# kscalelabs/kbot-joystick

Hardware: AMD Instinct MI355X
Metric: env-steps/sec (whole node), K-Bot joystick 8192 envs @1/2/4/8 MI355X (higher is better)
Workload: dtype f32; 1 GPU; kbot-headless, 8192 envs/GPU, flat ground, fixed joystick command (0.5,0,0), full iteration: 100-step rollout + PPO update (batch 512/GPU, 3 passes, LSTM hidden 256, depth 2); envs_per_gpu=8192, rollout_steps=100, batch_size_per_gpu=512, num_passes=3, hidden_size=256, deterministic_update=True, parallelism=env-sharded dp1, grad all-reduce per optimizer step

## Files before the change

### kbot-joystick_amd/csrc/kbj_gemm.h

```cpp
#pragma once
#include <hip/hip_runtime.h>
#include <algorithm>
#include <type_traits>
#include "kbj_ctx.h"

namespace kbj {

typedef float f32x16 __attribute__((ext_vector_type(16)));
typedef float f32x4 __attribute__((ext_vector_type(4)));

struct GemmArgs {
  const float* A; const float* B; float* C; const float* bias;
  int M, N, K;
  int lda, ldb, ldc;
  int beta;
  int splitk;
  const int* a_rows;
  const float* A2 = nullptr; const float* B2 = nullptr; int k1 = 0;
  float* C2 = nullptr; int n1 = 0, ldb2 = 0, ldc2 = 0;
  const int* a_idx = nullptr; int a_B = 0, a_N = 0;
  float* skws = nullptr;
  int x3 = 0;
};

constexpr int GEMM_BK = 32;
constexpr int GEMM_LDK = 36;

template <int ROWS, bool KC, int NTH>
struct GemmStage {
  static constexpr int NV = ROWS * 8 / NTH;
  static constexpr int RPP = NTH / 8;
  f32x4 v[NV];
  __device__ __forceinline__ void load_fast(const float* __restrict__ P, int ld, int r0, int k0) {
    const int tid = threadIdx.x;
    if (KC) {
      const int kq = tid & 7, rr = tid >> 3;
      const float* p = P + (size_t)(r0 + rr) * ld + k0 + 4 * kq;
#pragma unroll
      for (int i = 0; i < NV; ++i) v[i] = *reinterpret_cast<const f32x4*>(p + (size_t)(RPP * i) * ld);
    } else {
      constexpr int QPR = ROWS / 4, KROWS = NTH / QPR;
      const int rq = tid % QPR, kr0 = tid / QPR;
      const float* p = P + (size_t)(k0 + kr0) * ld + r0 + 4 * rq;
#pragma unroll
      for (int i = 0; i < NV; ++i) v[i] = *reinterpret_cast<const f32x4*>(p + (size_t)(KROWS * i) * ld);
    }
  }
  __device__ __forceinline__ void load(const float* __restrict__ P, int ld, int R, int r0, int k0, int kend, bool vec, const int* idx = nullptr, int iB = 0,
                                       int iN = 0) {
    const int tid = threadIdx.x;
    if (KC) {
      const int kq = tid & 7, rr = tid >> 3;
#pragma unroll
      for (int i = 0; i < NV; ++i) {
        int r = r0 + rr + RPP * i, k = k0 + 4 * kq;
        f32x4 x = {0, 0, 0, 0};
        if (r < R) {
          size_t base = (size_t)r * ld;
          if (idx) { const int t = r / iB; base = ((size_t)t * iN + idx[r - t * iB]) * ld; }
          if (vec && k + 3 < kend) x = *reinterpret_cast<const f32x4*>(P + base + k);
          else { for (int e = 0; e < 4; ++e) if (k + e < kend) x[e] = P[base + k + e]; }
        }
        v[i] = x;
      }
    } else {
      constexpr int QPR = ROWS / 4, KROWS = NTH / QPR;
      const int rq = tid % QPR, kr0 = tid / QPR;
#pragma unroll
      for (int i = 0; i < NV; ++i) {
        int k = k0 + kr0 + KROWS * i, r = r0 + 4 * rq;
        f32x4 x = {0, 0, 0, 0};
        if (k < kend) {
          size_t base = (size_t)k * ld;
          if (vec && r + 3 < R) x = *reinterpret_cast<const f32x4*>(P + base + r);
          else { for (int e = 0; e < 4; ++e) if (r + e < R) x[e] = P[base + r + e]; }
        }
        v[i] = x;
      }
    }
  }
  __device__ __forceinline__ void store(float* lds) const {
    const int tid = threadIdx.x;
    if (KC) {
      const int kq = tid & 7, rr = tid >> 3;
#pragma unroll
      for (int i = 0; i < NV; ++i) *reinterpret_cast<f32x4*>(lds + (rr + RPP * i) * GEMM_LDK + 4 * kq) = v[i];
    } else {
      constexpr int QPR = ROWS / 4, KROWS = NTH / QPR;
      const int rq = tid % QPR, kr0 = tid / QPR;
#pragma unroll
      for (int i = 0; i < NV; ++i) *reinterpret_cast<f32x4*>(lds + (kr0 + KROWS * i) * (ROWS + 4) + 4 * rq) = v[i];
    }
  }
};

struct GemmItem { int m0, n0, kbeg, kend, ks; const float* B; float* C; int ncols, ldb, ldc, ncol0; };
template <int BM, int BN>
__device__ __forceinline__ GemmItem gemm_item(const GemmArgs& g, int item, int tiles_n, int tiles_m, int per) {
  GemmItem it;
  int tn = item % tiles_n, r = item / tiles_n;
  int tm = r % tiles_m;
  it.ks = r / tiles_m;
  it.m0 = tm * BM; it.n0 = tn * BN;
  it.B = g.B; it.C = g.C; it.ncols = g.N; it.ldb = g.ldb; it.ldc = g.ldc; it.ncol0 = 0;
  if (g.n1 > 0) {
    if (it.n0 >= g.n1) {
      it.B = g.B2; it.C = g.C2; it.n0 -= g.n1; it.ncols = g.N - g.n1; it.ncol0 = g.n1;
      if (g.ldb2 > 0) it.ldb = g.ldb2;
      if (g.ldc2 > 0) it.ldc = g.ldc2;
    }
    else it.ncols = g.n1;
  }
  it.kbeg = it.ks * per;
  it.kend = min(g.K, it.kbeg + per);
  return it;
}

template <int MT, int NT, bool A_KC, bool B_KC, int WM = 2, int WN = 2>
__global__ __launch_bounds__(64 * WM * WN) void gemm_f32_kernel(GemmArgs g) {
  constexpr int BM = 32 * MT * WM, BN = 32 * NT * WN, NTH = 64 * WM * WN;
  constexpr int A_ELEMS = A_KC ? BM * GEMM_LDK : GEMM_BK * (BM + 4);
  constexpr int B_ELEMS = B_KC ? BN * GEMM_LDK : GEMM_BK * (BN + 4);
  constexpr int STAGE = A_ELEMS + B_ELEMS;
  extern __shared__ __attribute__((aligned(16))) float lds[];
  const int tid = threadIdx.x, lane = tid & 63, wave = tid >> 6;
  const int wr = wave / WN, wc = wave % WN;
  const int lr = lane & 31, lh = lane >> 5;
  const int tiles_n = (g.N + BN - 1) / BN, tiles_m = (g.M + BM - 1) / BM;
  const int sk = g.splitk > 1 ? g.splitk : 1;
  const int per = sk > 1 ? ((g.K + sk - 1) / sk + GEMM_BK - 1) / GEMM_BK * GEMM_BK : g.K;
  const int items = tiles_n * tiles_m * sk;
  const int item = (blockIdx.x & 7) * (gridDim.x >> 3) + (blockIdx.x >> 3);
  if (item >= items) return;
  const GemmItem cur = gemm_item<BM, BN>(g, item, tiles_n, tiles_m, per);
  if (cur.kbeg >= cur.kend) return;

  const bool a_vec = (g.lda & 3) == 0 && (((size_t)g.A & 15) == 0) && (((size_t)g.A2 & 15) == 0);
  const bool b_vec = (g.ldb & 3) == 0 && (g.ldb2 & 3) == 0 && (((size_t)g.B & 15) == 0) && (((size_t)g.B2 & 15) == 0);
  const bool rows_a = a_vec && cur.m0 + BM <= g.M, rows_b = b_vec && cur.n0 + BN <= cur.ncols;
  GemmStage<BM, A_KC, NTH> sa;
  GemmStage<BN, B_KC, NTH> sb;
  unsigned voa[GemmStage<BM, A_KC, NTH>::NV], vob[GemmStage<BN, B_KC, NTH>::NV];
  {
    if (A_KC) { const int kq = tid & 7, rr = tid >> 3;
#pragma unroll
      for (int i = 0; i < sa.NV; ++i) {
        size_t row = (size_t)(cur.m0 + rr + sa.RPP * i);
        if (g.a_idx && rows_a) {
          const int m = (int)row, t = m / g.a_B;
          row = (size_t)(t - cur.m0 / g.a_B) * g.a_N + g.a_idx[m - t * g.a_B];
        }
        voa[i] = (unsigned)((row * g.lda + 4 * kq) * 4);
      } }
    else { constexpr int QPR = BM / 4, KROWS = NTH / QPR; const int rq = tid % QPR, kr0 = tid / QPR;
#pragma unroll
      for (int i = 0; i < sa.NV; ++i) voa[i] = (unsigned)(((size_t)(kr0 + KROWS * i) * g.lda + cur.m0 + 4 * rq) * 4); }
    if (B_KC) { const int kq = tid & 7, rr = tid >> 3;
#pragma unroll
      for (int i = 0; i < sb.NV; ++i) vob[i] = (unsigned)(((size_t)(cur.n0 + rr + sb.RPP * i) * cur.ldb + 4 * kq) * 4); }
    else { constexpr int QPR = BN / 4, KROWS = NTH / QPR; const int rq = tid % QPR, kr0 = tid / QPR;
#pragma unroll
      for (int i = 0; i < sb.NV; ++i) vob[i] = (unsigned)(((size_t)(kr0 + KROWS * i) * cur.ldb + cur.n0 + 4 * rq) * 4); }
  }
  auto load_tile = [&](int k) {
    const float *pa = g.A, *pb = cur.B;
    int kk = k, ke = cur.kend;
    if (g.k1 > 0) {
      if (k >= g.k1) { pa = g.A2; pb = g.B2; kk = k - g.k1; ke = g.K - g.k1; }
      else ke = g.k1;
    }
    const bool kfull = kk + GEMM_BK <= ke;
    if (rows_a && kfull) {
      if (A_KC && g.a_idx) pa += (size_t)(cur.m0 / g.a_B) * g.a_N * g.lda;
      __amdgpu_buffer_rsrc_t ra = __builtin_amdgcn_make_buffer_rsrc(const_cast<float*>(pa), 0, 0x7FFFFFFF, 0x00020000);
      const unsigned so = (unsigned)(A_KC ? (size_t)kk * 4 : (size_t)kk * g.lda * 4);
#pragma unroll
      for (int i = 0; i < sa.NV; ++i) sa.v[i] = __builtin_bit_cast(f32x4, __builtin_amdgcn_raw_buffer_load_b128(ra, voa[i], so, 0));
    } else sa.load(pa, g.lda, g.M, cur.m0, kk, ke, a_vec, A_KC ? g.a_idx : nullptr, g.a_B, g.a_N);
    if (rows_b && kfull) {
      __amdgpu_buffer_rsrc_t rb = __builtin_amdgcn_make_buffer_rsrc(const_cast<float*>(pb), 0, 0x7FFFFFFF, 0x00020000);
      const unsigned so = (unsigned)(B_KC ? (size_t)kk * 4 : (size_t)kk * cur.ldb * 4);
#pragma unroll
      for (int i = 0; i < sb.NV; ++i) sb.v[i] = __builtin_bit_cast(f32x4, __builtin_amdgcn_raw_buffer_load_b128(rb, vob[i], so, 0));
    } else sb.load(pb, cur.ldb, cur.ncols, cur.n0, kk, ke, b_vec);
  };
  load_tile(cur.kbeg);
  sa.store(lds); sb.store(lds + A_ELEMS);
  __syncthreads();

  f32x16 acc[MT][NT];
#pragma unroll
  for (int i = 0; i < MT; ++i)
#pragma unroll
    for (int j = 0; j < NT; ++j)
#pragma unroll
      for (int r = 0; r < 16; ++r) acc[i][j][r] = 0.0f;

  auto k_tile = [&](auto stage_tag, int k0) {
    constexpr int S = decltype(stage_tag)::value;
    const bool more = k0 + GEMM_BK < cur.kend;
    if (more) load_tile(k0 + GEMM_BK);
    const float* As = lds + S * STAGE;
    const float* Bs = As + A_ELEMS;
#pragma unroll
    for (int half = 0; half < 2; ++half) {
#pragma unroll
      for (int kk = 2 * half; kk < 2 * half + 2; ++kk) {
        f32x4 a[MT], b[NT];
#pragma unroll
        for (int i = 0; i < MT; ++i) {
          int row = wr * 32 * MT + 32 * i + lr;
          if (A_KC) a[i] = *reinterpret_cast<const f32x4*>(As + row * GEMM_LDK + 8 * kk + 4 * lh);
          else { for (int e = 0; e < 4; ++e) a[i][e] = As[(8 * kk + 4 * lh + e) * (BM + 4) + row]; }
        }
#pragma unroll
        for (int j = 0; j < NT; ++j) {
          int row = wc * 32 * NT + 32 * j + lr;
          if (B_KC) b[j] = *reinterpret_cast<const f32x4*>(Bs + row * GEMM_LDK + 8 * kk + 4 * lh);
          else { for (int e = 0; e < 4; ++e) b[j][e] = Bs[(8 * kk + 4 * lh + e) * (BN + 4) + row]; }
        }
#pragma unroll
        for (int e = 0; e < 4; ++e)
#pragma unroll
          for (int i = 0; i < MT; ++i)
#pragma unroll
            for (int j = 0; j < NT; ++j) acc[i][j] = __builtin_amdgcn_mfma_f32_32x32x2f32(a[i][e], b[j][e], acc[i][j], 0, 0, 0);
      }
      if (half == 0 && more) {
        float* dst = lds + (S ^ 1) * STAGE;
        sa.store(dst); sb.store(dst + A_ELEMS);
      }
    }
    __syncthreads();
  };
  for (int k0 = cur.kbeg; k0 < cur.kend; k0 += 2 * GEMM_BK) {
    k_tile(std::integral_constant<int, 0>{}, k0);
    if (k0 + GEMM_BK < cur.kend) k_tile(std::integral_constant<int, 1>{}, k0 + GEMM_BK);
  }
#pragma unroll
  for (int i = 0; i < MT; ++i)
#pragma unroll
    for (int j = 0; j < NT; ++j) {
      int n = cur.n0 + wc * 32 * NT + 32 * j + lr;
      if (n >= cur.ncols) continue;
      float bv = (g.bias && cur.ks == 0) ? g.bias[n] : 0.0f;
#pragma unroll
      for (int r = 0; r < 16; ++r) {
        int m = cur.m0 + wr * 32 * MT + 32 * i + (r & 3) + 8 * (r >> 2) + 4 * lh;
        if (m >= g.M) continue;
        float* c = cur.C + (size_t)m * cur.ldc + n;
        float v = acc[i][j][r] + bv;
#ifdef KBJ_GEMM_NOSTORE
        if (v == 1.2345e-30f) *c = v;
#else
        if (sk > 1) {
          if (g.skws) g.skws[((size_t)cur.ks * g.M + m) * g.N + cur.ncol0 + n] = v;
          else atomicAdd(c, v);
        } else *c = g.beta ? *c + v : v;
#endif
      }
    }
}


typedef short bf16x8 __attribute__((ext_vector_type(8)));
typedef unsigned u32x2 __attribute__((ext_vector_type(2)));
constexpr int X3_LD = 40;
constexpr int X3_PIECE = 128 * X3_LD;
__device__ __forceinline__ void x3_split(const f32x4& x, u32x2& hi, u32x2& mid, u32x2& lo) {
  unsigned h[4], m[4], l[4];
#pragma unroll
  for (int e = 0; e < 4; ++e) {
    h[e] = __float_as_uint(x[e]) & 0xFFFF0000u;
    const float r1 = x[e] - __uint_as_float(h[e]);
    m[e] = __float_as_uint(r1) & 0xFFFF0000u;
    l[e] = __float_as_uint(r1 - __uint_as_float(m[e]));
  }
  hi = {__builtin_amdgcn_perm(h[1], h[0], 0x07060302u), __builtin_amdgcn_perm(h[3], h[2], 0x07060302u)};
  mid = {__builtin_amdgcn_perm(m[1], m[0], 0x07060302u), __builtin_amdgcn_perm(m[3], m[2], 0x07060302u)};
  lo = {__builtin_amdgcn_perm(l[1], l[0], 0x07060302u), __builtin_amdgcn_perm(l[3], l[2], 0x07060302u)};
}
template <bool KC, int ROWS> struct X3Stage {
  static constexpr int NG = ROWS / 32;
  static_assert(KC || ROWS == 128, "row-contiguous operands are transposed in 4 x 4 blocks: 128-row tiles only");
  f32x4 v[NG];
  __device__ __forceinline__ void load(const float* __restrict__ P, int ld, int R, int r0, int k0) {
    const int t = threadIdx.x;
    if (KC) { const int kq = t & 7, rr = t >> 3;
#pragma unroll
      for (int i = 0; i < NG; ++i) {
        const int r = r0 + rr + 32 * i;
        v[i] = r < R ? *reinterpret_cast<const f32x4*>(P + (size_t)r * ld + k0 + 4 * kq) : f32x4{0, 0, 0, 0};
      }
    } else { const int kg = t & 7, rq = t >> 3, r = r0 + 4 * rq;
      f32x4 w[4];
#pragma unroll
      for (int j = 0; j < 4; ++j) {
        const float* p = P + (size_t)(k0 + 4 * kg + j) * ld + r;
        if (r + 3 < R) w[j] = *reinterpret_cast<const f32x4*>(p);
        else { for (int e = 0; e < 4; ++e) w[j][e] = r + e < R ? p[e] : 0.0f; }
      }
#pragma unroll
      for (int i = 0; i < 4; ++i) v[i] = {w[0][i], w[1][i], w[2][i], w[3][i]};
    }
  }
  __device__ __forceinline__ void load_gen(const float* __restrict__ P, const long (&roff)[NG], int k0, int kend) {
    const int k = k0 + 4 * (threadIdx.x & 7);
#pragma unroll
    for (int i = 0; i < NG; ++i) v[i] = (roff[i] >= 0 && k + 3 < kend) ? *reinterpret_cast<const f32x4*>(P + roff[i] + k) : f32x4{0, 0, 0, 0};
  }
  __device__ __forceinline__ void store(short* lds) const {
    const int t = threadIdx.x;
#pragma unroll
    for (int i = 0; i < NG; ++i) {
      const int row = KC ? (t >> 3) + 32 * i : 4 * (t >> 3) + i, k = 4 * (t & 7);
      u32x2 hi, mid, lo;
      x3_split(v[i], hi, mid, lo);
      short* p = lds + row * X3_LD + k;
      *reinterpret_cast<u32x2*>(p) = hi; *reinterpret_cast<u32x2*>(p + ROWS * X3_LD) = mid; *reinterpret_cast<u32x2*>(p + 2 * ROWS * X3_LD) = lo;
    }
  }
};
template <int TM, bool A_KC, bool B_KC, bool GEN>
__global__ __launch_bounds__(256, 2) void gemm_x3_kernel(GemmArgs g) {
  constexpr int BM = 64 * TM, PIECE = BM * X3_LD;
  static_assert(!GEN || (A_KC && B_KC), "the general loads are written for k-contiguous operands");
  extern __shared__ __attribute__((aligned(16))) short x3lds[];
  short* As = x3lds; short* Bs = x3lds + 3 * PIECE;
  const int lane = threadIdx.x & 63, wave = threadIdx.x >> 6, wr = wave >> 1, wc = wave & 1, lr = lane & 31, lh = lane >> 5;
  const int tiles_n = (g.N + BM - 1) / BM, tiles_m = (g.M + BM - 1) / BM;
  const int sk = g.splitk > 1 ? g.splitk : 1;
  const int per = sk > 1 ? ((g.K + sk - 1) / sk + GEMM_BK - 1) / GEMM_BK * GEMM_BK : g.K;
  const int item = (blockIdx.x & 7) * (gridDim.x >> 3) + (blockIdx.x >> 3);
  if (item >= tiles_n * tiles_m * sk) return;
  const GemmItem cur = gemm_item<BM, BM>(g, item, tiles_n, tiles_m, per);
  if (cur.kbeg >= cur.kend) return;
  X3Stage<A_KC, BM> sa; X3Stage<B_KC, BM> sb;
  long roa[X3Stage<A_KC, BM>::NG], rob[X3Stage<B_KC, BM>::NG];
  if (GEN) {
#pragma unroll
    for (int i = 0; i < sa.NG; ++i) {
      const int m = cur.m0 + (threadIdx.x >> 3) + 32 * i, n = cur.n0 + (threadIdx.x >> 3) + 32 * i;
      long row = m;
      if (g.a_idx && m < g.M) { const int tt = m / g.a_B; row = (long)tt * g.a_N + g.a_idx[m - tt * g.a_B]; }
      roa[i] = m < g.M ? row * g.lda : -1;
      rob[i] = n < cur.ncols ? (long)n * cur.ldb : -1;
    }
  }
  auto load_tile = [&](int k) {
    if (GEN) {
      const float *pa = g.A, *pb = cur.B;
      int kk = k, ke = cur.kend;
      if (g.k1 > 0) { if (k >= g.k1) { pa = g.A2; pb = g.B2; kk = k - g.k1; ke = g.K - g.k1; } else ke = g.k1; }
      sa.load_gen(pa, roa, kk, ke); sb.load_gen(pb, rob, kk, ke);
    } else { sa.load(g.A, g.lda, g.M, cur.m0, k); sb.load(cur.B, cur.ldb, cur.ncols, cur.n0, k); }
  };
  load_tile(cur.kbeg);
  f32x16 acc[TM][TM];
#pragma unroll
  for (int i = 0; i < TM; ++i)
#pragma unroll
    for (int j = 0; j < TM; ++j)
#pragma unroll
      for (int r = 0; r < 16; ++r) acc[i][j][r] = 0.0f;
  for (int k0 = cur.kbeg; k0 < cur.kend; k0 += 32) {
    __syncthreads();
    sa.store(As); sb.store(Bs);
    __syncthreads();
    if (k0 + 32 < cur.kend) load_tile(k0 + 32);
#pragma unroll
    for (int kk = 0; kk < 2; ++kk) {
      bf16x8 a[3][TM], b[3][TM];
#pragma unroll
      for (int p = 0; p < 3; ++p)
#pragma unroll
        for (int i = 0; i < TM; ++i) {
          a[p][i] = *reinterpret_cast<const bf16x8*>(As + p * PIECE + (wr * 32 * TM + 32 * i + lr) * X3_LD + 16 * kk + 8 * lh);
          b[p][i] = *reinterpret_cast<const bf16x8*>(Bs + p * PIECE + (wc * 32 * TM + 32 * i + lr) * X3_LD + 16 * kk + 8 * lh);
        }
      constexpr int PA[6] = {1, 2, 0, 1, 0, 0}, PB[6] = {1, 0, 2, 0, 1, 0};
#pragma unroll
      for (int q = 0; q < 6; ++q)
#pragma unroll
        for (int i = 0; i < TM; ++i)
#pragma unroll
          for (int j = 0; j < TM; ++j) acc[i][j] = __builtin_amdgcn_mfma_f32_32x32x16_bf16(a[PA[q]][i], b[PB[q]][j], acc[i][j], 0, 0, 0);
    }
  }
#pragma unroll
  for (int i = 0; i < TM; ++i)
#pragma unroll
    for (int j = 0; j < TM; ++j) {
      const int n = cur.n0 + wc * 32 * TM + 32 * j + lr;
      if (n >= cur.ncols) continue;
      const float bv = (GEN && g.bias && cur.ks == 0) ? g.bias[n] : 0.0f;
#pragma unroll
      for (int r = 0; r < 16; ++r) {
        const int m = cur.m0 + wr * 32 * TM + 32 * i + (r & 3) + 8 * (r >> 2) + 4 * lh;
        if (m >= g.M) continue;
        float* c = cur.C + (size_t)m * cur.ldc + n;
        const float v = acc[i][j][r] + bv;
        if (sk > 1) atomicAdd(c, v);
        else *c = g.beta ? *c + v : v;
      }
    }
}
inline int gemm_x3_form(const GemmArgs& g, bool a_kc, bool b_kc, bool big) {
  if (!g.x3 || g.skws || (g.B2 && g.n1 <= 0 && g.k1 <= 0)) return 0;
  auto al = [](const void* p, int ld) { return ((size_t)p & 15) == 0 && (ld & 3) == 0; };
  if (!al(g.A, g.lda) || !al(g.B, g.ldb) || g.M < 64 || g.N < 64) return 0;
  const bool gen = g.bias || g.k1 > 0 || g.a_idx || g.K % GEMM_BK != 0;
  if (gen) {
    if (!a_kc || !b_kc || g.n1 > 0 || g.splitk > 1 || g.K % 4 != 0 || g.k1 % GEMM_BK != 0) return 0;
    if (g.k1 > 0 && (!al(g.A2, g.lda) || !al(g.B2, g.ldb))) return 0;
    return 2;
  }
  if (!big && !(a_kc && b_kc)) return 0;
  if (g.n1 > 0 && (!al(g.B2, g.ldb2 > 0 ? g.ldb2 : g.ldb) || g.n1 % (big ? 128 : 64) != 0)) return 0;
  return 1;
}
template <int TM, bool A_KC, bool B_KC, bool GEN> inline void gemm_x3_launch_tile(hipStream_t s, const GemmArgs& g, int sk) {
  constexpr int BM = 64 * TM;
  constexpr size_t bytes = 6 * BM * X3_LD * sizeof(short);
  static const hipError_t attr = hipFuncSetAttribute(reinterpret_cast<const void*>(&gemm_x3_kernel<TM, A_KC, B_KC, GEN>), hipFuncAttributeMaxDynamicSharedMemorySize, (int)bytes);
  (void)attr;
  const long it = (long)((g.M + BM - 1) / BM) * ((g.N + BM - 1) / BM) * sk;
  KbjKernelTimer timer(s, kbj_kind_gemm_x3(TM, A_KC, B_KC, GEN), 2.0 * g.M * g.N * g.K);
  hipLaunchKernelGGL((gemm_x3_kernel<TM, A_KC, B_KC, GEN>), dim3((unsigned)((it + 7) / 8 * 8)), dim3(256), bytes, s, g);
}

__global__ void splitk_reduce_kernel(GemmArgs g, int sk, int per) {
  const size_t i = (size_t)blockIdx.x * blockDim.x + threadIdx.x;
  if (i >= (size_t)g.M * g.N) return;
  const int m = (int)(i / g.N), n = (int)(i % g.N);
  const int full = (g.K + per - 1) / per, nks = sk < full ? sk : full;
  const size_t stride = (size_t)g.M * g.N;
  const float* p = g.skws + i;
  float* c = (g.n1 > 0 && n >= g.n1) ? g.C2 + (size_t)m * (g.ldc2 > 0 ? g.ldc2 : g.ldc) + (n - g.n1) : g.C + (size_t)m * g.ldc + n;
  const float c0 = *c;
  float s = 0.0f;
  for (int k0 = 0; k0 < nks; k0 += 8) {
    float v[8];
#pragma unroll
    for (int j = 0; j < 8; ++j) v[j] = p[(size_t)(k0 + j < nks ? k0 + j : nks - 1) * stride];
#pragma unroll
    for (int j = 0; j < 8; ++j) if (k0 + j < nks) s += v[j];
  }
  *c = c0 + s;
}

inline void splitk_reduce_launch(hipStream_t s, const GemmArgs& g, int sk) {
  const int per = ((g.K + sk - 1) / sk + GEMM_BK - 1) / GEMM_BK * GEMM_BK;
  hipLaunchKernelGGL(splitk_reduce_kernel, dim3((unsigned)(((size_t)g.M * g.N + 255) / 256)), dim3(256), 0, s, g, sk, per);
}

template <int MT, int NT, bool A_KC, bool B_KC, int WM = 2, int WN = 2>
inline void gemm_launch_tile(hipStream_t s, const GemmArgs& g, int wgs) {
  constexpr int BM = 32 * MT * WM, BN = 32 * NT * WN;
  constexpr size_t bytes = 2 * sizeof(float) * ((A_KC ? BM * GEMM_LDK : GEMM_BK * (BM + 4)) + (B_KC ? BN * GEMM_LDK : GEMM_BK * (BN + 4)));
  static const hipError_t attr = hipFuncSetAttribute(reinterpret_cast<const void*>(&gemm_f32_kernel<MT, NT, A_KC, B_KC, WM, WN>),
                                                      hipFuncAttributeMaxDynamicSharedMemorySize, (int)bytes);
  (void)attr;
  hipLaunchKernelGGL((gemm_f32_kernel<MT, NT, A_KC, B_KC, WM, WN>), dim3(wgs), dim3(64 * WM * WN), bytes, s, g);
}

template <bool A_KC, bool B_KC>
inline void gemm_launch(hipStream_t s, const GemmArgs& g_in, int force_big = -1) {
  GemmArgs g = g_in;
  int sk = g.splitk > 1 ? g.splitk : 1;
  long big_items = (long)((g.M + 127) / 128) * ((g.N + 127) / 128) * sk;
  bool big = force_big >= 0 ? force_big != 0 : (big_items >= 192 && g.N > 64);
  long items = big ? big_items : (long)((g.M + 63) / 64) * ((g.N + 63) / 64) * sk;
  int wgs = (int)items;
  wgs = (wgs + 7) / 8 * 8;
  if (const int form = gemm_x3_form(g, A_KC, B_KC, big)) {
    if constexpr (A_KC && B_KC) {
      if (form == 2) { if (big) gemm_x3_launch_tile<2, true, true, true>(s, g, sk); else gemm_x3_launch_tile<1, true, true, true>(s, g, sk); }
      else { if (big) gemm_x3_launch_tile<2, true, true, false>(s, g, sk); else gemm_x3_launch_tile<1, true, true, false>(s, g, sk); }
    } else gemm_x3_launch_tile<2, A_KC, B_KC, false>(s, g, sk);
    return;
  }
  if constexpr (A_KC) {
    if (force_big == 2 && sk == 1) {
      KbjKernelTimer timer(s, KBJ_KIND_GEMM_64x128 + (B_KC ? 0 : 1), 2.0 * g.M * g.N * g.K);
      const long it = (long)((g.M + 63) / 64) * ((g.N + 127) / 128);
      gemm_launch_tile<1, 1, true, B_KC, 2, 4>(s, g, (int)((it + 7) / 8 * 8));
      return;
    }
  }
  KbjKernelTimer timer(s, KBJ_KIND_GEMM + (big ? 0 : 4) + (A_KC ? 2 : 0) + (B_KC ? 1 : 0), 2.0 * g.M * g.N * g.K);
#ifdef KBJ_GEMM_W4
  if (big) gemm_launch_tile<2, 2, A_KC, B_KC>(s, g, wgs);
#else
  if (big) gemm_launch_tile<2, 1, A_KC, B_KC, 2, 4>(s, g, wgs);
#endif
  else gemm_launch_tile<1, 1, A_KC, B_KC>(s, g, wgs);
  if (sk > 1 && g.skws) splitk_reduce_launch(s, g, sk);
}

}
```

Before: 2.333 million env-steps/s.

## Remap waves for ragged N tiles and use bounded buffer loads for partial B

For the 2x4-wave fp32 MFMA GEMM configuration, when the last N tile has fewer than four 32-column blocks, the waves are remapped so all of them cover the occupied column blocks instead of idle waves issuing MFMAs on padding. The K loop is specialized per active block count so waves with no work skip MFMAs. Partial B tiles also get a buffer resource with a bounded record size, so they can use the fast buffer-load path with hardware out-of-bounds zeroing instead of the slow guarded scalar path. This adds code-size and branch complexity, and relies on buffer OOB semantics for correctness on the ragged edge.

```diff
diff --git a/kbot-joystick_amd/csrc/kbj_gemm.h b/kbot-joystick_amd/csrc/kbj_gemm.h
--- a/kbot-joystick_amd/csrc/kbj_gemm.h
+++ b/kbot-joystick_amd/csrc/kbj_gemm.h
@@ -21,10 +21,16 @@
   const int* a_idx = nullptr; int a_B = 0, a_N = 0;
   float* skws = nullptr;
   int x3 = 0;
+  int ragged_off = 0;
 };
+#ifndef KBJ_GEMM_RAGGED_OFF
+#define KBJ_GEMM_RAGGED_OFF 0
+#endif
 
 constexpr int GEMM_BK = 32;
 constexpr int GEMM_LDK = 36;
+
+__host__ __device__ inline size_t gemm_rowc_extent(int K, int ld) { return (size_t)K * (size_t)ld * sizeof(float); }
 
 template <int ROWS, bool KC, int NTH>
 struct GemmStage {
@@ -138,6 +144,23 @@
   const bool a_vec = (g.lda & 3) == 0 && (((size_t)g.A & 15) == 0) && (((size_t)g.A2 & 15) == 0);
   const bool b_vec = (g.ldb & 3) == 0 && (g.ldb2 & 3) == 0 && (((size_t)g.B & 15) == 0) && (((size_t)g.B2 & 15) == 0);
   const bool rows_a = a_vec && cur.m0 + BM <= g.M, rows_b = b_vec && cur.n0 + BN <= cur.ncols;
+  const int ragged_off = g.ragged_off | KBJ_GEMM_RAGGED_OFF;
+  bool rag_b = false;
+  if constexpr (!B_KC) rag_b = b_vec && !rows_b && !(ragged_off & 1) && gemm_rowc_extent(g.K, cur.ldb) <= 0x7FFFFFFFu;
+  constexpr bool RAGMAP = MT == 2 && NT == 1 && WM == 2 && WN == 4 && !A_KC && !B_KC;
+  int row0 = wr * 32 * MT, col0 = wc * 32 * NT, nblk = MT;
+  if constexpr (RAGMAP) {
+    const int c = (min(cur.ncols - cur.n0, BN) + 31) >> 5;
+    if (c < 4 && !(ragged_off & 2)) {
+      const int w = __builtin_amdgcn_readfirstlane(wave);
+      if (c == 3) {
+        if (w < 3) { row0 = 0; col0 = 32 * w; nblk = 2; }
+        else if (w == 3) { row0 = 64; col0 = 0; nblk = 2; }
+        else { row0 = 64 + 32 * (w & 1); col0 = 32 * (1 + ((w - 4) >> 1)); nblk = 1; }
+      } else if (c == 2) { row0 = 32 * (w >> 1); col0 = 32 * (w & 1); nblk = 1; }
+      else { row0 = 32 * (w & 3); col0 = 0; nblk = w < 4 ? 1 : 0; }
+    }
+  }
   GemmStage<BM, A_KC, NTH> sa;
   GemmStage<BN, B_KC, NTH> sb;
   unsigned voa[GemmStage<BM, A_KC, NTH>::NV], vob[GemmStage<BN, B_KC, NTH>::NV];
@@ -177,9 +200,12 @@
 #pragma unroll
       for (int i = 0; i < sa.NV; ++i) sa.v[i] = __builtin_bit_cast(f32x4, __builtin_amdgcn_raw_buffer_load_b128(ra, voa[i], so, 0));
     } else sa.load(pa, g.lda, g.M, cur.m0, kk, ke, a_vec, A_KC ? g.a_idx : nullptr, g.a_B, g.a_N);
-    if (rows_b && kfull) {
-      __amdgpu_buffer_rsrc_t rb = __builtin_amdgcn_make_buffer_rsrc(const_cast<float*>(pb), 0, 0x7FFFFFFF, 0x00020000);
-      const unsigned so = (unsigned)(B_KC ? (size_t)kk * 4 : (size_t)kk * cur.ldb * 4);
+    if ((rows_b || rag_b) && kfull) {
+      unsigned so = (unsigned)(B_KC ? (size_t)kk * 4 : (size_t)kk * cur.ldb * 4), rec = 0x7FFFFFFFu;
+      if (rag_b) {
+        pb += (size_t)kk * cur.ldb; rec = (unsigned)gemm_rowc_extent(g.K - kk, cur.ldb); so = 0;
+      }
+      __amdgpu_buffer_rsrc_t rb = __builtin_amdgcn_make_buffer_rsrc(const_cast<float*>(pb), 0, (int)rec, 0x00020000);
 #pragma unroll
       for (int i = 0; i < sb.NV; ++i) sb.v[i] = __builtin_bit_cast(f32x4, __builtin_amdgcn_raw_buffer_load_b128(rb, vob[i], so, 0));
     } else sb.load(pb, cur.ldb, cur.ncols, cur.n0, kk, ke, b_vec);
@@ -196,8 +222,8 @@
 #pragma unroll
       for (int r = 0; r < 16; ++r) acc[i][j][r] = 0.0f;
 
-  auto k_tile = [&](auto stage_tag, int k0) {
-    constexpr int S = decltype(stage_tag)::value;
+  auto k_tile = [&](auto stage_tag, auto nb_tag, int k0) {
+    constexpr int S = decltype(stage_tag)::value, NB = decltype(nb_tag)::value;
     const bool more = k0 + GEMM_BK < cur.kend;
     if (more) load_tile(k0 + GEMM_BK);
     const float* As = lds + S * STAGE;
@@ -208,21 +234,21 @@
       for (int kk = 2 * half; kk < 2 * half + 2; ++kk) {
         f32x4 a[MT], b[NT];
 #pragma unroll
-        for (int i = 0; i < MT; ++i) {
-          int row = wr * 32 * MT + 32 * i + lr;
+        for (int i = 0; i < NB; ++i) {
+          int row = row0 + 32 * i + lr;
           if (A_KC) a[i] = *reinterpret_cast<const f32x4*>(As + row * GEMM_LDK + 8 * kk + 4 * lh);
           else { for (int e = 0; e < 4; ++e) a[i][e] = As[(8 * kk + 4 * lh + e) * (BM + 4) + row]; }
         }
 #pragma unroll
-        for (int j = 0; j < NT; ++j) {
-          int row = wc * 32 * NT + 32 * j + lr;
+        for (int j = 0; j < (NB ? NT : 0); ++j) {
+          int row = col0 + 32 * j + lr;
           if (B_KC) b[j] = *reinterpret_cast<const f32x4*>(Bs + row * GEMM_LDK + 8 * kk + 4 * lh);
           else { for (int e = 0; e < 4; ++e) b[j][e] = Bs[(8 * kk + 4 * lh + e) * (BN + 4) + row]; }
         }
 #pragma unroll
         for (int e = 0; e < 4; ++e)
 #pragma unroll
-          for (int i = 0; i < MT; ++i)
+          for (int i = 0; i < NB; ++i)
 #pragma unroll
             for (int j = 0; j < NT; ++j) acc[i][j] = __builtin_amdgcn_mfma_f32_32x32x2f32(a[i][e], b[j][e], acc[i][j], 0, 0, 0);
       }
@@ -233,20 +259,27 @@
     }
     __syncthreads();
   };
-  for (int k0 = cur.kbeg; k0 < cur.kend; k0 += 2 * GEMM_BK) {
-    k_tile(std::integral_constant<int, 0>{}, k0);
-    if (k0 + GEMM_BK < cur.kend) k_tile(std::integral_constant<int, 1>{}, k0 + GEMM_BK);
-  }
+  auto k_loop = [&](auto nb_tag) {
+    for (int k0 = cur.kbeg; k0 < cur.kend; k0 += 2 * GEMM_BK) {
+      k_tile(std::integral_constant<int, 0>{}, nb_tag, k0);
+      if (k0 + GEMM_BK < cur.kend) k_tile(std::integral_constant<int, 1>{}, nb_tag, k0 + GEMM_BK);
+    }
+  };
+  if constexpr (RAGMAP) {
+    if (nblk == 2) k_loop(std::integral_constant<int, 2>{});
+    else if (nblk == 1) k_loop(std::integral_constant<int, 1>{});
+    else k_loop(std::integral_constant<int, 0>{});
+  } else k_loop(std::integral_constant<int, MT>{});
 #pragma unroll
   for (int i = 0; i < MT; ++i)
 #pragma unroll
     for (int j = 0; j < NT; ++j) {
-      int n = cur.n0 + wc * 32 * NT + 32 * j + lr;
-      if (n >= cur.ncols) continue;
+      int n = cur.n0 + col0 + 32 * j + lr;
+      if (i >= nblk || n >= cur.ncols) continue;
       float bv = (g.bias && cur.ks == 0) ? g.bias[n] : 0.0f;
 #pragma unroll
       for (int r = 0; r < 16; ++r) {
-        int m = cur.m0 + wr * 32 * MT + 32 * i + (r & 3) + 8 * (r >> 2) + 4 * lh;
+        int m = cur.m0 + row0 + 32 * i + (r & 3) + 8 * (r >> 2) + 4 * lh;
         if (m >= g.M) continue;
         float* c = cur.C + (size_t)m * cur.ldc + n;
         float v = acc[i][j][r] + bv;
```

Result: no change. 2.346 million env-steps/s, median of 6 (+0.5%).
